# ikt-luh/Demo-Learned-Point-Cloud-Compression

Hardware: AMD Instinct MI355X
Metric: point-cloud frames/sec encode+decode @1M pts (higher is better)
Workload: dtype f32

## Files before the change

### demo-learned-point-cloud-compression_amd/csrc/codec.hip

```cpp
#include "common.h"

#include <string.h>

#include <algorithm>
#include <atomic>
#include <chrono>
#include <deque>
#include <exception>
#include <new>
#include <map>
#include <memory>
#include <string>
#include <condition_variable>
#include <functional>
#include <mutex>
#include <thread>
#include <vector>

namespace {

double now_s() {
  return std::chrono::duration<double>(std::chrono::steady_clock::now().time_since_epoch()).count();
}

// ... 652 lines not shown
};

int rans_encode_grow(const int32_t* sym, const int32_t* idx, int64_t n, const Tensor* cdf, const Tensor* len,
                     const Tensor* off, std::vector<uint8_t>* out) {
  int64_t cap = 2 * n + 4096, got = 0;
  int rc = PCC_OK;
  for (int attempt = 0; attempt < 2; ++attempt) {
    out->resize((size_t)cap);
    rc = pcc_rans_encode(sym, idx, n, cdf->i32(), (int)cdf->dims[1], len->i32(), off->i32(), (int)cdf->dims[0],
                         out->data(), cap, &got);
    if (rc != PCC_E_NOMEM) break;
    cap = 48 * n + 4096;
  }
  if (rc == PCC_OK) out->resize((size_t)got);
  return rc;
}

}


static void warm_copy_paths(pcc_codec* cd) {
  hipStream_t st = cd->ctx->stream;
  const size_t big = (size_t)1 << 20;
  uint8_t *d = nullptr, *h = nullptr;
  if (hipMalloc((void**)&d, 2 * big) != hipSuccess) return;
  if (hipHostMalloc((void**)&h, 2 * big, hipHostMallocDefault) == hipSuccess) {
    for (int rep = 0; rep < 2; ++rep) {
      for (size_t bytes : {(size_t)64, (size_t)4096, (size_t)65536, big}) {
        for (int k = 0; k < 4; ++k) {
          (void)hipMemcpyAsync(h + (size_t)k * (big / 4), d + (size_t)k * (big / 4), std::min(bytes, big / 4), hipMemcpyDeviceToHost, st);
          (void)hipMemcpyAsync(d + big + (size_t)k * (big / 4), h + big + (size_t)k * (big / 4), std::min(bytes, big / 4),
                               hipMemcpyHostToDevice, st);
        }
        (void)hipMemcpy2DAsync(h, big / 4, d, big / 4, std::min(bytes, big / 4), 3, hipMemcpyDeviceToHost, st);
        (void)hipMemcpy2DAsync(h + big, big / 4, d + big, big / 4, std::min(bytes, big / 4) / 2 + 1, 3, hipMemcpyDeviceToHost, st);
      }
      (void)hipMemsetAsync(d, 0, 4096, st);
      (void)hipMemcpyAsync(d + big, d, 65536, hipMemcpyDeviceToDevice, st);
    }
    (void)hipStreamSynchronize(st);
    (void)hipHostFree(h);
  }
  (void)hipFree(d);
  (void)hipGetLastError();
}

extern "C" pcc_codec* pcc_codec_create(const void* h_ckpt, size_t n, int device, void* stream) {
  if (!h_ckpt || n < 8 || memcmp(h_ckpt, "PCCW", 4) != 0) {
    pcc_set_error("pcc_codec_create: not a PCCW checkpoint blob");
    return nullptr;
  }
  pcc_ctx* ctx = pcc_create(device, stream);
  if (!ctx) return nullptr;
  pcc_codec* cd = new pcc_codec();
  cd->ctx = ctx;
  cd->device = device;
  cd->blob.assign((const uint8_t*)h_ckpt, (const uint8_t*)h_ckpt + n);
  const uint8_t* p = cd->blob.data();
  size_t pos = 4;
  auto fail = [&](const char* why) -> pcc_codec* {
    pcc_set_error("pcc_codec_create: malformed checkpoint (%s)", why);
    pcc_destroy(cd->ctx);
    delete cd;
    return nullptr;
  };
  uint32_t count;
  memcpy(&count, p + pos, 4);
  pos += 4;
  for (uint32_t i = 0; i < count; ++i) {
// ... 508 lines not shown
    return PCC_OK;
  }
};

struct EncodeCall {
  pcc_codec* cd;
  pcc_ctx* ctx;
  hipStream_t st;
  const double* h_q;
  int n_frames, n_q, cy, cz;
  bool v1 = false;
  pcc_ctx* side = nullptr;
  double ts[8] = {0, 0, 0, 0, 0, 0, 0, 0};
  Feat x, y, z, z_hat, gp;
  View yv, zv;
  int64_t ny = 0, nz = 0;
  float* ys_f = nullptr;
  int32_t* zsym_dev = nullptr;
  const std::vector<int64_t>* yoffs = nullptr;
  std::vector<uint64_t> root_keys;
  std::vector<int64_t> counts[3];
  GeoSlotEncoder geo;
  int64_t cap_y = 0, cap_z = 0;
  long long* d_lens = nullptr;
  hipEvent_t z_done = nullptr;
  const Tensor *eb_cdf = nullptr, *eb_len = nullptr, *eb_off = nullptr;
  const Tensor *gc_cdf = nullptr, *gc_len = nullptr, *gc_off = nullptr;
  std::vector<std::vector<uint8_t>> blobs, y_strings;
  std::vector<uint8_t> z_string, head_done;
  std::vector<int64_t> seek_idx;
  std::vector<std::vector<uint64_t>> seek_state;
  std::vector<std::vector<int64_t>> seek_word;
  int n_chunks = 1;
  std::vector<int64_t> bound;
  std::vector<hipEvent_t> evc;
  std::vector<int> rcq;
  std::vector<std::string> errq;
  double helper_z_s = 0;
  EncodeCall(pcc_codec* c, int nf, const double* q, int nq)
      : cd(c), ctx(c->ctx), st(c->ctx->stream), h_q(q), n_frames(nf), n_q(nq), cy(c->c_y), cz(c->c_z),
        blobs((size_t)nf), y_strings((size_t)nq), head_done((size_t)nq, 0) {}
  int unpack(int64_t n, const int32_t* d_coords, const float* d_feats, const FrameTab* frames_in, const HostFrames* host) {
    CODEC_ALLOC(keys, uint64_t, n);
    CODEC_ALLOC(flag, int32_t, 1);
    CODEC_ALLOC(perm, uint32_t, n);
    CODEC_ALLOC(f, float, 4 * n);
    PCC_HIP(hipMemsetAsync(flag, 0, 4, st));
    FrameTab ftab;
    const FrameTab* frames = frames_in;
    std::vector<UploadPiece> col_pieces;
    std::atomic<int> up_status{0};
    WorkersGuard up_guard{nullptr};
    if (host) {
      if (!cd->up_stream) {
        PCC_HIP(hipStreamCreateWithFlags(&cd->up_stream, hipStreamNonBlocking));
        PCC_HIP(hipEventCreateWithFlags(&cd->up_done, hipEventDisableTiming));
      }
      PCC_HIP(hipStreamSynchronize(cd->up_stream));
      ftab = *frames_in;
      const size_t pb = ftab.pts_i16 ? 6 : 12, cb = 12;
      char* dp = (char*)cd->pool.alloc((size_t)n * pb + 256 * (size_t)ftab.nf);
      char* dc = (char*)cd->pool.alloc((size_t)n * cb + 256 * (size_t)ftab.nf);
      if (!dp || !dc) return PCC_E_NOMEM;
      std::vector<UploadPiece> pt_pieces;
      size_t po = 0, co = 0;
      for (int f = 0; f < ftab.nf; ++f) {
// ... 168 lines not shown
    for (int attempt = 0; attempt < 2; ++attempt) {
      if (attempt == 1) {
        cap_y = pcc_rans_dev_bound(per);
        cap_z = pcc_rans_dev_bound(nzs);
      }
      PCC_TRY(cd->pin_ysym.ensure((size_t)cap_y * n_q + (size_t)cap_z + 256));
      ystreams = cd->pin_ysym.p;
      zstream = cd->pin_ysym.p + (size_t)cap_y * n_q;
      PCC_TRY(pcc_rans_encode_dev_async(ctx, cd->gc_dev, sym32, idx8, 1, per, n_q, ystreams, cap_y, d_lens, attempt));
      if (attempt == 0 && z_done)
        PCC_HIP(hipStreamWaitEvent(st, z_done, 0));
      else
        PCC_TRY(pcc_rans_encode_dev_async(ctx, cd->eb_dev, zsym_dev, nullptr, std::max<int64_t>(nz, 1), nzs, 1, zstream, cap_z,
                                          d_lens + n_q, attempt));
      PCC_HIP(hipMemcpyAsync(h_lens, d_lens, (size_t)(n_q + 1) * 8, hipMemcpyDeviceToHost, st));
      if (attempt == 0) PCC_TRY(geo.finish(true, blobs));
      PCC_HIP(hipStreamSynchronize(st));
      bool fits = true;
      for (int q = 0; q <= n_q; ++q) fits &= h_lens[q] >= 0;
      if (fits) break;
      PCC_REQUIRE(attempt == 0, PCC_E_NOMEM, "pcc_encode_gop: a coded stream exceeds its bound");
    }
    for (int q = 0; q < n_q; ++q) y_strings[q].assign(ystreams + (size_t)q * cap_y, ystreams + (size_t)q * cap_y + h_lens[q]);
    z_string.assign(zstream, zstream + h_lens[n_q]);
    return PCC_OK;
  }
  int gaussian_v0(float* params, float* scale_d, const Tensor* tab) {
    gc_cdf = find(cd, "gaussian_conditional.quantized_cdf");
    gc_len = find(cd, "gaussian_conditional.cdf_length");
    gc_off = find(cd, "gaussian_conditional.offset");
    PCC_REQUIRE(tab && gc_cdf && gc_len && gc_off, PCC_E_ARG, "pcc_encode_gop: gaussian_conditional tables missing");
    const int ntab = (int)tab->dims[0];
    const int64_t per = (int64_t)cy * ny, tot = per * n_q;
    CODEC_ALLOC(sym16, int16_t, std::max<int64_t>(tot, 1));
    CODEC_ALLOC(idx8, uint8_t, std::max<int64_t>(tot, 1));
    CODEC_ALLOC(flag, int32_t, 1);
    PCC_TRY(cd->pin_ysym.ensure((size_t)std::max<int64_t>(tot, 1) * 4));
    PCC_TRY(cd->pin_yidx.ensure((size_t)std::max<int64_t>(tot, 1) * 4));
    PCC_HIP(hipMemsetAsync(flag, 0, 4, st));
    if (ny > 0)
      PCC_TRY(pcc_gaussian_quant16(ctx, ys_f, params, ny, cy, scale_d, n_q, cd->dev["gaussian_conditional.scale_table"],
                                   ntab, sym16, idx8, flag));
    PCC_HIP(hipMemcpyAsync(cd->pin_flag.p, flag, 4, hipMemcpyDeviceToHost, st));
    n_chunks = per >= (1 << 16) ? 4 : 1;
    bound.resize((size_t)n_chunks);
    for (int c = 0; c < n_chunks; ++c) bound[c] = (per * (n_chunks - 1 - c) / n_chunks) & ~(int64_t)63;
    evc.assign((size_t)n_chunks, nullptr);
    for (int c = 0; c < n_chunks; ++c) {
      const int64_t lo = bound[c], hi = c == 0 ? per : bound[c - 1];
      if (ny > 0 && hi > lo) {
        PCC_HIP(hipMemcpy2DAsync(cd->pin_ysym.p + (size_t)lo * 2, (size_t)per * 2, sym16 + lo, (size_t)per * 2,
                                 (size_t)(hi - lo) * 2, (size_t)n_q, hipMemcpyDeviceToHost, st));
        PCC_HIP(hipMemcpy2DAsync(cd->pin_yidx.p + (size_t)lo, (size_t)per, idx8 + lo, (size_t)per, (size_t)(hi - lo),
                                 (size_t)n_q, hipMemcpyDeviceToHost, st));
      }
      PCC_TRY(call_event(cd, &evc[c]));
      PCC_HIP(hipEventRecord(evc[c], st));
    }
    rcq.assign((size_t)n_q, PCC_OK);
    errq.assign((size_t)n_q, std::string());
    seek_indexes(per, cd->seek_points, &seek_idx);
    seek_state.assign((size_t)n_q, std::vector<uint64_t>(seek_idx.size() + 1, 0));
    seek_word.assign((size_t)n_q, std::vector<int64_t>(seek_idx.size() + 1, 0));
    int side_rc = PCC_OK;
    {
      WorkersGuard wait_all{&cd->workers};
      cd->workers.ensure(n_q);
      for (int q = 0; q < n_q; ++q) cd->workers.run(q, [this, q]() { code_quality(q); });
      side_rc = geometry_and_z();
    }
    PCC_TRY(side_rc);
    for (int q = 0; q < n_q; ++q)
      if (rcq[q] != PCC_OK) {
        pcc_set_error("pcc_encode_gop (y stream %d): %s", q, errq[q].c_str());
        return rcq[q];
      }
    if (*(int32_t*)cd->pin_flag.p == 0) return PCC_OK;
    return gaussian_int32(params, scale_d, ntab);
  }
  void code_quality(int q) {
    struct GateUser {
      hipEvent_t* ev;
      bool failed;
    };
    (void)hipSetDevice(cd->device);
    GateUser gu{evc.data(), false};
    PccRansGate gate{n_chunks, bound.data(),
                     [](void* u, int c) {
                       GateUser* g = (GateUser*)u;
                       if (hipEventSynchronize(g->ev[c]) != hipSuccess) g->failed = true;
                     },
                     &gu};
    gate.fn(&gu, 0);
    if (gu.failed) {
      rcq[q] = PCC_E_HIP;
      errq[q] = "hipEventSynchronize failed";
      return;
    }
    if (*(volatile int32_t*)cd->pin_flag.p != 0) return;
    const int64_t per = (int64_t)cy * ny;
    int64_t capq = 2 * per + 4096, got = 0;
    std::unique_ptr<uint8_t[]> ybuf;
    for (int attempt = 0; attempt < 2; ++attempt) {
      ybuf.reset(new uint8_t[(size_t)capq]);
      PccRansSeek seek{(int)seek_idx.size(), seek_idx.data(), seek_state[q].data(), seek_word[q].data()};
      rcq[q] = pcc_rans_encode16_seek((const int16_t*)cd->pin_ysym.p + (size_t)q * per, cd->pin_yidx.p + (size_t)q * per,
                                      per, gc_cdf->i32(), (int)gc_cdf->dims[1], gc_len->i32(), gc_off->i32(),
                                      (int)gc_cdf->dims[0], ybuf.get(), capq, &got, &gate, cd->gc_tables,
                                      seek_idx.empty() ? nullptr : &seek);
      if (rcq[q] != PCC_E_NOMEM) break;
      capq = 48 * per + 4096;
    }
    if (rcq[q] == PCC_OK && gu.failed) {
      rcq[q] = PCC_E_HIP;
      errq[q] = "hipEventSynchronize failed";
    } else if (rcq[q] == PCC_OK) {
      std::vector<uint8_t>& o = cd->out[q];
      o.clear();
      o.reserve((size_t)got + 65536);
      put_head(o, n_frames, q, got, 0);
      o.insert(o.end(), ybuf.get(), ybuf.get() + got);
      head_done[q] = 1;
    } else {
      errq[q] = pcc_last_error();
    }
  }
  int geometry_and_z() {
    PCC_TRY(geo.device_half(ctx));
    PCC_TRY(geo.finish(false, blobs));
    double t = now_s();
    std::vector<int32_t> idx((size_t)nz * cz);
    for (int c = 0; c < cz; ++c) std::fill(idx.begin() + (size_t)c * nz, idx.begin() + (size_t)(c + 1) * nz, c);
    PCC_TRY(rans_encode_grow((const int32_t*)cd->pin_zsym.p, idx.data(), nz * cz, eb_cdf, eb_len, eb_off, &z_string));
    helper_z_s = now_s() - t;
    return PCC_OK;
  }
  int gaussian_int32(const float* params, const float* scale_d, int ntab) {
    const int64_t per = (int64_t)cy * ny, tot = per * n_q;
    int64_t cap = 2 * per + 4096;
    std::fill(head_done.begin(), head_done.end(), 0);
    CODEC_ALLOC(sym32, int32_t, std::max<int64_t>(tot, 1));
    CODEC_ALLOC(idx32, int32_t, std::max<int64_t>(tot, 1));
// ... 991 lines not shown
```

### demo-learned-point-cloud-compression_amd/csrc/entropy.hip

```cpp
#include "common.h"

__global__ __launch_bounds__(256) void k_factorized_quant(const float* __restrict__ z, int64_t n, int c,
                                                          const float* __restrict__ med,
                                                          int32_t* __restrict__ sym,
                                                          float* __restrict__ zhat) {
  const int64_t t = (int64_t)blockIdx.x * blockDim.x + threadIdx.x;
  if (t >= n * c) return;
  const int ch = (int)(t / n);
  const int64_t i = t - (int64_t)ch * n;
  const float m = med[ch];
  const float r = rintf(__fsub_rn(z[i * c + ch], m));
  sym[t] = (int32_t)r;
  zhat[i * c + ch] = __fadd_rn(r, m);
}

__global__ __launch_bounds__(256) void k_factorized_dequant(const int32_t* __restrict__ sym, int64_t n,
                                                            int c, const float* __restrict__ med,
                                                            float* __restrict__ zhat) {
  const int64_t t = (int64_t)blockIdx.x * blockDim.x + threadIdx.x;
  if (t >= n * c) return;
  const int ch = (int)(t / n);
  const int64_t i = t - (int64_t)ch * n;
  zhat[i * c + ch] = __fadd_rn((float)sym[t], med[ch]);
}

__device__ __forceinline__ int32_t scale_index(float sc, const float* __restrict__ table, int n_tab) {
  const float s = fmaxf(sc, table[0]);
  int32_t idx = n_tab - 1;
  for (int j = 0; j < n_tab - 1; ++j) idx -= (s <= table[j]) ? 1 : 0;
  return idx;
}

constexpr int GQ_TILE = 16;
constexpr int GQ_MAX_C = 256;
static inline size_t gq_lds_bytes(int c, int planes) { return (size_t)(64 + planes * GQ_TILE * (c + 1)) * 4; }

__device__ __forceinline__ void gq_stage(const float* __restrict__ src, int64_t row0, int rows, int width, int col0, int c,
                                         float* __restrict__ dst) {
  const int lane = threadIdx.x & 63, wave = threadIdx.x >> 6, nw = blockDim.x >> 6;
  for (int r = wave; r < rows; r += nw) {
    const float* row = src + (row0 + r) * width + col0;
    for (int j = lane; j < c; j += 64) dst[r * (c + 1) + j] = row[j];
  }
}

__device__ __forceinline__ bool gq_load_table(const float* __restrict__ table, int n_tab, float* __restrict__ tab) {
  if (threadIdx.x < n_tab) tab[threadIdx.x] = table[threadIdx.x];
  __syncthreads();
  const bool ok = !((int)threadIdx.x + 1 < n_tab) || tab[threadIdx.x] <= tab[threadIdx.x + 1];
  return __syncthreads_and(ok) != 0;
}
__device__ __forceinline__ int32_t scale_index_fast(float sc, const float* __restrict__ tab, int n_tab, bool ascending) {
  if (!ascending) return scale_index(sc, tab, n_tab);
  const float s = fmaxf(sc, tab[0]);
  int lo = 0, hi = n_tab - 1;
  while (lo < hi) {
    const int mid = (lo + hi) >> 1;
    if (tab[mid] >= s) hi = mid;
    else lo = mid + 1;
  }
  return lo;
}

template <typename SymT, typename IdxT, bool CHECK16>
__global__ __launch_bounds__(256) void k_gaussian_quant_t(
    const float* __restrict__ y, const float* __restrict__ params, int64_t n, int c,
    const float* __restrict__ scale, int nq, const float* __restrict__ table, int n_tab,
    SymT* __restrict__ sym, IdxT* __restrict__ idx, int32_t* __restrict__ flag) {
  extern __shared__ float gq_lds[];
  float* tab = gq_lds;
  float* yt = gq_lds + 64;
  float* sct = yt + GQ_TILE * (c + 1);
  float* mut = sct + GQ_TILE * (c + 1);
  const bool asc = gq_load_table(table, n_tab, tab);
  const int64_t row0 = (int64_t)blockIdx.x * GQ_TILE;
  const int rows = (int)min((int64_t)GQ_TILE, n - row0);
  gq_stage(y, row0, rows, c, 0, c, yt);
  gq_stage(params, row0, rows, 2 * c, 0, c, sct);
  gq_stage(params, row0, rows, 2 * c, c, c, mut);
  __syncthreads();
  bool over = false;
  for (int e = threadIdx.x; e < GQ_TILE * c; e += blockDim.x) {
    const int ch = e / GQ_TILE, r = e - ch * GQ_TILE;
    if (r >= rows) continue;
    const float yv = yt[r * (c + 1) + ch], sc = sct[r * (c + 1) + ch], mu = mut[r * (c + 1) + ch];
    const int64_t t = (int64_t)ch * n + row0 + r;
    for (int q = 0; q < nq; ++q) {
      const float s = scale[q * c + ch];
      const float v = rintf(__fsub_rn(__fmul_rn(yv, s), __fmul_rn(mu, s)));
      if constexpr (CHECK16) over |= !(v >= -32768.0f && v <= 32767.0f);
      sym[(int64_t)q * n * c + t] = (SymT)(int32_t)v;
      idx[(int64_t)q * n * c + t] = (IdxT)scale_index_fast(__fmul_rn(sc, s), tab, n_tab, asc);
    }
  }
  if constexpr (CHECK16)
    if (over) atomicOr(flag, 1);
}

template <typename IdxT>
__global__ __launch_bounds__(256) void k_gaussian_indexes_t(const float* __restrict__ params, int64_t n, int c,
                                                            const float* __restrict__ scale,
                                                            const float* __restrict__ table, int n_tab,
                                                            IdxT* __restrict__ idx) {
  extern __shared__ float gq_lds[];
  float* tab = gq_lds;
  float* sct = gq_lds + 64;
  const bool asc = gq_load_table(table, n_tab, tab);
  const int64_t row0 = (int64_t)blockIdx.x * GQ_TILE;
  const int rows = (int)min((int64_t)GQ_TILE, n - row0);
  gq_stage(params, row0, rows, 2 * c, 0, c, sct);
  __syncthreads();
  for (int e = threadIdx.x; e < GQ_TILE * c; e += blockDim.x) {
    const int ch = e / GQ_TILE, r = e - ch * GQ_TILE;
    if (r >= rows) continue;
    idx[(int64_t)ch * n + row0 + r] = (IdxT)scale_index_fast(__fmul_rn(sct[r * (c + 1) + ch], scale[ch]), tab, n_tab, asc);
  }
}

__global__ __launch_bounds__(256) void k_gaussian_dequant(const int32_t* __restrict__ sym,
                                                          const float* __restrict__ params, int64_t n,
                                                          int c, const float* __restrict__ scale,
                                                          float bound, float off_a, float off_b,
                                                          float* __restrict__ yhat) {
  extern __shared__ float gq_lds[];
  float* sct = gq_lds + 64;
// ... 87 lines not shown
                     c, d_med, d_zhat);
  PCC_CHECK_LAUNCH();
  return PCC_OK;
}

extern "C" int pcc_gaussian_quant(pcc_ctx* ctx, const float* d_y, const float* d_params, int64_t n,
                                  int c, const float* d_scale, int q, const float* d_table, int n_tab,
                                  int32_t* d_sym, int32_t* d_idx) {
  PCC_REQUIRE(ctx && c >= 1 && c <= GQ_MAX_C && q >= 1 && n_tab >= 2 && n_tab <= 64, PCC_E_ARG,
              "pcc_gaussian_quant: bad arg (c=%d q=%d n_tab=%d)", c, q, n_tab);
  if (n <= 0) return PCC_OK;
  PCC_REQUIRE(d_y && d_params && d_scale && d_table && d_sym && d_idx, PCC_E_ARG,
              "pcc_gaussian_quant: null buffers");
  hipLaunchKernelGGL((k_gaussian_quant_t<int32_t, int32_t, false>), dim3(nblk(n, GQ_TILE)), dim3(256), gq_lds_bytes(c, 3),
                     ctx->stream, d_y, d_params, n, c, d_scale, q, d_table, n_tab, d_sym, d_idx, (int32_t*)nullptr);
  PCC_CHECK_LAUNCH();
  return PCC_OK;
}

extern "C" int pcc_gaussian_quant16(pcc_ctx* ctx, const float* d_y, const float* d_params, int64_t n,
                                    int c, const float* d_scale, int q, const float* d_table, int n_tab,
                                    int16_t* d_sym, uint8_t* d_idx, int32_t* d_flag) {
  PCC_REQUIRE(ctx && c >= 1 && c <= GQ_MAX_C && q >= 1 && n_tab >= 2 && n_tab <= 64, PCC_E_ARG,
              "pcc_gaussian_quant16: bad arg (c=%d q=%d n_tab=%d)", c, q, n_tab);
  if (n <= 0) return PCC_OK;
  PCC_REQUIRE(d_y && d_params && d_scale && d_table && d_sym && d_idx && d_flag, PCC_E_ARG,
              "pcc_gaussian_quant16: null buffers");
  hipLaunchKernelGGL((k_gaussian_quant_t<int16_t, uint8_t, true>), dim3(nblk(n, GQ_TILE)), dim3(256), gq_lds_bytes(c, 3),
                     ctx->stream, d_y, d_params, n, c, d_scale, q, d_table, n_tab, d_sym, d_idx, d_flag);
  PCC_CHECK_LAUNCH();
  return PCC_OK;
}

extern "C" int pcc_gaussian_quant_dev(pcc_ctx* ctx, const float* d_y, const float* d_params, int64_t n, int c,
                                      const float* d_scale, int q, const float* d_table, int n_tab, int32_t* d_sym,
                                      uint8_t* d_idx) {
  PCC_REQUIRE(ctx && c >= 1 && c <= GQ_MAX_C && q >= 1 && n_tab >= 2 && n_tab <= 64, PCC_E_ARG,
              "pcc_gaussian_quant_dev: bad arg (c=%d q=%d n_tab=%d)", c, q, n_tab);
  if (n <= 0) return PCC_OK;
  PCC_REQUIRE(d_y && d_params && d_scale && d_table && d_sym && d_idx, PCC_E_ARG, "pcc_gaussian_quant_dev: null buffers");
  hipLaunchKernelGGL((k_gaussian_quant_t<int32_t, uint8_t, false>), dim3(nblk(n, GQ_TILE)), dim3(256), gq_lds_bytes(c, 3),
                     ctx->stream, d_y, d_params, n, c, d_scale, q, d_table, n_tab, d_sym, d_idx, (int32_t*)nullptr);
  PCC_CHECK_LAUNCH();
  return PCC_OK;
}

extern "C" int pcc_gaussian_indexes8(pcc_ctx* ctx, const float* d_params, int64_t n, int c,
                                     const float* d_scale, const float* d_table, int n_tab,
                                     uint8_t* d_idx) {
  PCC_REQUIRE(ctx && c >= 1 && c <= GQ_MAX_C && n_tab >= 2 && n_tab <= 64, PCC_E_ARG, "pcc_gaussian_indexes8: bad arg");
  if (n <= 0) return PCC_OK;
  PCC_REQUIRE(d_params && d_scale && d_table && d_idx, PCC_E_ARG, "pcc_gaussian_indexes8: null buffers");
  hipLaunchKernelGGL((k_gaussian_indexes_t<uint8_t>), dim3(nblk(n, GQ_TILE)), dim3(256), gq_lds_bytes(c, 1), ctx->stream,
                     d_params, n, c, d_scale, d_table, n_tab, d_idx);
  PCC_CHECK_LAUNCH();
  return PCC_OK;
}

extern "C" int pcc_gaussian_indexes(pcc_ctx* ctx, const float* d_params, int64_t n, int c,
                                    const float* d_scale, const float* d_table, int n_tab,
                                    int32_t* d_idx) {
  PCC_REQUIRE(ctx && c >= 1 && c <= GQ_MAX_C && n_tab >= 2 && n_tab <= 64, PCC_E_ARG, "pcc_gaussian_indexes: bad arg");
  if (n <= 0) return PCC_OK;
  PCC_REQUIRE(d_params && d_scale && d_table && d_idx, PCC_E_ARG, "pcc_gaussian_indexes: null buffers");
  hipLaunchKernelGGL((k_gaussian_indexes_t<int32_t>), dim3(nblk(n, GQ_TILE)), dim3(256), gq_lds_bytes(c, 1), ctx->stream,
                     d_params, n, c, d_scale, d_table, n_tab, d_idx);
// ... 16 lines not shown
```

### demo-learned-point-cloud-compression_amd/csrc/rans_gate.h

```cpp
#pragma once
#include <stdint.h>
#include <vector>

struct PccRansGate {
  int n_chunks;
  const int64_t* bound;
  void (*fn)(void* user, int chunk);
  void* user;
};
struct PccRansTables;
PccRansTables* pcc_rans_tables_build(const int32_t* h_cdfs, int cdf_pitch, const int32_t* h_sizes,
                                     const int32_t* h_offsets, int n_cdf);
void pcc_rans_tables_free(PccRansTables* t);
int pcc_rans_encode16_gated(const int16_t* h_sym, const uint8_t* h_idx, int64_t n, const int32_t* h_cdfs,
                            int cdf_pitch, const int32_t* h_sizes, const int32_t* h_offsets, int n_cdf,
                            uint8_t* h_out, int64_t cap, int64_t* h_len, const PccRansGate* gate,
                            const PccRansTables* tables);
struct PccRansSeek {
  int n;
  const int64_t* index;
  uint64_t* state;
  int64_t* word;
};
int pcc_rans_encode16_seek(const int16_t* h_sym, const uint8_t* h_idx, int64_t n, const int32_t* h_cdfs,
                           int cdf_pitch, const int32_t* h_sizes, const int32_t* h_offsets, int n_cdf,
                           uint8_t* h_out, int64_t cap, int64_t* h_len, const PccRansGate* gate,
                           const PccRansTables* tables, PccRansSeek* seek);
int pcc_rans_decode8_range(const uint8_t* h_in, int64_t len, const uint8_t* h_idx, int64_t n, const int32_t* h_cdfs,
                           int cdf_pitch, const int32_t* h_sizes, const int32_t* h_offsets, int n_cdf, int32_t* h_sym,
                           const PccRansTables* tables, int64_t i_lo, int64_t i_hi, uint64_t state_in, int64_t word_in,
                           uint64_t* state_out, int64_t* word_out);
int pcc_rans_decode8_gated(const uint8_t* h_in, int64_t len, const uint8_t* h_idx, int64_t n, const int32_t* h_cdfs,
                           int cdf_pitch, const int32_t* h_sizes, const int32_t* h_offsets, int n_cdf,
                           int32_t* h_sym, const PccRansGate* gate, const PccRansTables* tables);


int pcc_octree_unpack_vec(const uint8_t* h_in, int64_t len, std::vector<int32_t>* pts, int64_t* h_level_n);
struct PccOctPart {
  std::vector<uint64_t> cells;
  int64_t level_n[16];
};
int pcc_octree_parts(const uint8_t* h_in, int64_t len, int* K, const uint8_t** part, int64_t* part_len);
int pcc_octree_unpack_part(const uint8_t* h_in, int64_t len, PccOctPart* out);
int pcc_octree_merge_parts(const uint8_t* h_in, int64_t len, PccOctPart* parts, int K, std::vector<uint64_t>* cells,
                           int64_t* h_level_n);
void pcc_octree_cells_to_points(const uint64_t* cells, int64_t n, const int32_t origin[3], int32_t* out);
int pcc_octree_join_parts(int depth, const int32_t origin[3], int64_t n_points, const std::vector<uint8_t>* parts, int K,
                          uint8_t* h_out, int64_t cap, int64_t* h_len);

struct pcc_ctx;
struct pcc_rans_dev;
int pcc_rans_encode_dev_async(pcc_ctx* ctx, const pcc_rans_dev* tables, const int32_t* d_sym, const uint8_t* d_idx,
                              int64_t idx_run, int64_t n, int n_streams, uint8_t* d_out, int64_t cap_each,
                              long long* d_lens, int attempt);

int pcc_octree2_encode(pcc_ctx* ctx, const uint64_t* d_keys, int64_t n, int key_shift, int depth, const int32_t origin[3],
                       uint8_t* h_out, int64_t cap, int64_t* h_len);
int pcc_octree2_decode(pcc_ctx* ctx, const uint8_t* h_in, int64_t len, int32_t* d_points, int32_t* h_points, int64_t cap_points,
                       int64_t* h_n_points, int64_t* h_level_n);
```

### demo-learned-point-cloud-compression_amd/csrc/rans_host.cpp

```cpp
#include <stdint.h>
#include <string.h>
#include <stdio.h>
#include <algorithm>
#include <memory>
#include <thread>
#include <vector>
#include "../../include/pcc.h"
#include "rans_gate.h"

void pcc_set_error(const char* fmt, ...);

namespace {

constexpr uint32_t kPrecision = 16;
constexpr uint32_t kBypassBits = 4;
constexpr uint32_t kMaxBypass = (1u << kBypassBits) - 1;
constexpr uint64_t kRansL = 1ull << 31;

struct Enc {
  uint64_t x;
  uint32_t* ptr;
  uint32_t* floor;
  bool overflow;

// ... 44 lines not shown
      return PCC_E_ARG;
    }
    t->base[c + 1] = t->base[c] + sizes[c] - 1;
  }
  t->ent.resize((size_t)t->base[n_cdf]);
  for (int c = 0; c < n_cdf; ++c) {
    const int32_t* cdf = cdfs + (int64_t)c * pitch;
    for (int v = 0; v < sizes[c] - 1; ++v) {
      EncSym& e = t->ent[(size_t)t->base[c] + v];
      const int64_t f = (int64_t)cdf[v + 1] - cdf[v];
      e.freq = (f >= 1 && f <= 65536) ? (uint32_t)f : 0u;
      e.bias = (uint32_t)cdf[v];
      e.cmpl = (1u << kPrecision) - e.freq;
      if (e.freq < 2) {
        e.rcp = ~0ull;
        e.rs = 0;
        e.bias += (1u << kPrecision) - 1;
      } else {
        uint32_t shift = 0;
        while (e.freq > (1u << shift)) ++shift;
        e.rcp = (uint64_t)((((unsigned __int128)1 << (shift + 63)) + e.freq - 1) / e.freq);
        e.rs = shift - 1;
      }
      e.x_max = ((kRansL >> kPrecision) << 32) * (uint64_t)e.freq;
    }
  }
  return PCC_OK;
}

template <typename SymT, typename IdxT>
int encode_stream(const SymT* sym, const IdxT* idx, int64_t n, const int32_t* cdfs, int pitch,
                  const int32_t* sizes, const int32_t* offsets, int n_cdf, uint8_t* out, int64_t cap,
                  int64_t* len, char* err, size_t errlen, const PccRansGate* gate = nullptr,
                  const EncTables* pre = nullptr, PccRansSeek* seek = nullptr) {
  size_t buf_words = (size_t)(n / 2 + n / 8) + 1024;
  std::unique_ptr<uint32_t[]> buf(new uint32_t[buf_words]);
  EncTables local;
  if (!pre) {
    const int rc = build_enc_tables(cdfs, pitch, sizes, n_cdf, &local, err, errlen);
    if (rc != PCC_OK) return rc;
    pre = &local;
  }
  const std::vector<int32_t>& base = pre->base;
  const std::vector<EncSym>& ent = pre->ent;
  for (int attempt = 0; attempt < 3; ++attempt) {
    Enc e;
    e.x = kRansL;
    e.floor = buf.get();
    e.ptr = buf.get() + buf_words;
    e.overflow = false;
    const int n_chunks = gate ? gate->n_chunks : 1;
    int sk = seek ? seek->n - 1 : -1;
    while (sk >= 0 && seek->index[sk] >= n) --sk;
    for (int ch = 0; ch < n_chunks; ++ch) {
    const int64_t c_hi = (ch == 0 ? n : gate->bound[ch - 1]) - 1, c_lo = gate ? gate->bound[ch] : 0;
    if (gate) gate->fn(gate->user, ch);
    for (int64_t i_hi = c_hi; i_hi >= c_lo;) {
    const int64_t i_lo = (sk >= 0 && seek->index[sk] > c_lo) ? std::min<int64_t>(seek->index[sk], i_hi + 1) : c_lo;
    for (int64_t i = i_hi; i >= i_lo; --i) {
      const int32_t ci = (int32_t)idx[i];
      if ((uint32_t)ci >= (uint32_t)n_cdf) {
        snprintf(err, errlen, "rans encode: index %d out of range at %lld", ci, (long long)i);
        return PCC_E_ARG;
      }
      const int32_t max_value = sizes[ci] - 2;
      int32_t value = (int32_t)sym[i] - offsets[ci];
      if ((uint32_t)value >= (uint32_t)max_value) {
        uint32_t raw;
        if (value < 0) raw = (uint32_t)(-2 * (int64_t)value - 1);
        else raw = (uint32_t)(2 * ((int64_t)value - max_value));
        value = max_value;
        const int nb = n_nibbles(raw);
        for (int j = nb - 1; j >= 0; --j) e.put_bits((raw >> (j * kBypassBits)) & kMaxBypass);
        const int full = nb / (int)kMaxBypass;
        e.put_bits((uint32_t)(nb - full * (int)kMaxBypass));
        for (int j = 0; j < full; ++j) e.put_bits(kMaxBypass);
      }
      const EncSym& es = ent[(size_t)base[ci] + value];
      if (es.freq == 0) {
        snprintf(err, errlen, "rans encode: zero frequency (cdf %d, value %d)", ci, value);
        return PCC_E_ARG;
      }
      e.put(es);
    }
    while (sk >= 0 && seek->index[sk] >= i_lo && seek->index[sk] > 0) {
      seek->state[sk] = e.x;
      seek->word[sk] = (int64_t)((buf.get() + buf_words) - e.ptr);
      --sk;
    }
    i_hi = i_lo - 1;
    }
    }
    e.emit((uint32_t)(e.x >> 32));
    e.emit((uint32_t)(e.x >> 0));
    if (e.overflow) {
      buf_words = (size_t)n * 12 + 1024;
      buf.reset(new uint32_t[buf_words]);
      continue;
    }
// ... 253 lines not shown
      cdf_pitch < 2 || n_cdf < 1 || !gate_ok(gate, n, true)) {
    pcc_set_error("pcc_rans_encode16_gated: bad argument");
    return PCC_E_ARG;
  }
  char err[256] = {0};
  const int rc = encode_stream(h_sym, h_idx, n, h_cdfs, cdf_pitch, h_sizes, h_offsets, n_cdf, h_out, cap, h_len, err,
                               sizeof(err), gate, tables ? &tables->enc : nullptr);
  if (rc != PCC_OK) pcc_set_error("pcc_rans_encode16_gated: %s", err);
  return rc;
}

int pcc_rans_encode16_seek(const int16_t* h_sym, const uint8_t* h_idx, int64_t n, const int32_t* h_cdfs,
                           int cdf_pitch, const int32_t* h_sizes, const int32_t* h_offsets, int n_cdf,
                           uint8_t* h_out, int64_t cap, int64_t* h_len, const PccRansGate* gate,
                           const PccRansTables* tables, PccRansSeek* seek) {
  if (!h_len || n < 0 || (n > 0 && (!h_sym || !h_idx)) || !h_cdfs || !h_sizes || !h_offsets || !h_out ||
      cdf_pitch < 2 || n_cdf < 1 || !gate_ok(gate, n, true)) {
    pcc_set_error("pcc_rans_encode16_seek: bad argument");
    return PCC_E_ARG;
  }
  if (seek)
    for (int k = 0; k < seek->n; ++k)
      if (!seek->index || !seek->state || !seek->word || (k > 0 && seek->index[k] < seek->index[k - 1])) {
        pcc_set_error("pcc_rans_encode16_seek: seek indexes must ascend");
        return PCC_E_ARG;
      }
  char err[256] = {0};
  const int rc = encode_stream(h_sym, h_idx, n, h_cdfs, cdf_pitch, h_sizes, h_offsets, n_cdf, h_out, cap, h_len, err,
                               sizeof(err), gate, tables ? &tables->enc : nullptr, seek);
  if (rc != PCC_OK) pcc_set_error("pcc_rans_encode16_seek: %s", err);
  return rc;
}

int pcc_rans_decode8_range(const uint8_t* h_in, int64_t len, const uint8_t* h_idx, int64_t n, const int32_t* h_cdfs,
                           int cdf_pitch, const int32_t* h_sizes, const int32_t* h_offsets, int n_cdf, int32_t* h_sym,
                           const PccRansTables* tables, int64_t i_lo, int64_t i_hi, uint64_t state_in, int64_t word_in,
                           uint64_t* state_out, int64_t* word_out) {
  if (!tables || !state_out || !word_out || !h_in || len < 8) {
    pcc_set_error("pcc_rans_decode8_range: bad argument");
    return PCC_E_ARG;
  }
  DecPos from{state_in, word_in}, to{0, 0};
  if (i_lo == 0 && word_in == 0) {
    uint32_t w[2];
    memcpy(w, h_in, 8);
    from.x = (uint64_t)w[0] | ((uint64_t)w[1] << 32);
    from.word = 2;
  }
  const int rc = decode_stream(h_in, len, h_idx, n, h_cdfs, cdf_pitch, h_sizes, h_offsets, n_cdf, h_sym,
                               "pcc_rans_decode8_range", nullptr, &tables->dec, i_lo, i_hi, &from, &to);
  *state_out = to.x;
  *word_out = to.word;
  return rc;
}

int pcc_rans_decode8_gated(const uint8_t* h_in, int64_t len, const uint8_t* h_idx, int64_t n, const int32_t* h_cdfs,
                           int cdf_pitch, const int32_t* h_sizes, const int32_t* h_offsets, int n_cdf,
                           int32_t* h_sym, const PccRansGate* gate, const PccRansTables* tables) {
  if (!gate_ok(gate, n, false)) {
    pcc_set_error("pcc_rans_decode8_gated: bad chunk table");
    return PCC_E_ARG;
  }
  return decode_stream(h_in, len, h_idx, n, h_cdfs, cdf_pitch, h_sizes, h_offsets, n_cdf, h_sym,
                       "pcc_rans_decode8", gate, tables ? &tables->dec : nullptr);
}

// ... 82 lines not shown
```

Baseline: 118.8.

## Write gaussian symbols in chunk-contiguous pieces to replace strided 2D D2H copies

```diff
diff --git a/demo-learned-point-cloud-compression_amd/csrc/codec.hip b/demo-learned-point-cloud-compression_amd/csrc/codec.hip
--- a/demo-learned-point-cloud-compression_amd/csrc/codec.hip
+++ b/demo-learned-point-cloud-compression_amd/csrc/codec.hip
@@ -708,9 +708,8 @@
           (void)hipMemcpyAsync(d + big + (size_t)k * (big / 4), h + big + (size_t)k * (big / 4), std::min(bytes, big / 4),
                                hipMemcpyHostToDevice, st);
         }
-        (void)hipMemcpy2DAsync(h, big / 4, d, big / 4, std::min(bytes, big / 4), 3, hipMemcpyDeviceToHost, st);
-        (void)hipMemcpy2DAsync(h + big, big / 4, d + big, big / 4, std::min(bytes, big / 4) / 2 + 1, 3, hipMemcpyDeviceToHost, st);
-      }
+      }
+      (void)hipMemcpyAsync(h, d, 2 * big, hipMemcpyDeviceToHost, st);
       (void)hipMemsetAsync(d, 0, 4096, st);
       (void)hipMemcpyAsync(d + big, d, 65536, hipMemcpyDeviceToDevice, st);
     }
@@ -1285,6 +1284,7 @@
   std::vector<std::vector<uint64_t>> seek_state;
   std::vector<std::vector<int64_t>> seek_word;
   int n_chunks = 1;
+  PccSymPieces pieces{};
   std::vector<int64_t> bound;
   std::vector<hipEvent_t> evc;
   std::vector<int> rcq;
@@ -1519,28 +1519,31 @@
     PCC_REQUIRE(tab && gc_cdf && gc_len && gc_off, PCC_E_ARG, "pcc_encode_gop: gaussian_conditional tables missing");
     const int ntab = (int)tab->dims[0];
     const int64_t per = (int64_t)cy * ny, tot = per * n_q;
-    CODEC_ALLOC(sym16, int16_t, std::max<int64_t>(tot, 1));
-    CODEC_ALLOC(idx8, uint8_t, std::max<int64_t>(tot, 1));
+    n_chunks = per >= (1 << 16) ? 4 : 1;
+    bound.resize((size_t)n_chunks);
+    for (int c = 0; c < n_chunks; ++c) bound[c] = (per * (n_chunks - 1 - c) / n_chunks) & ~(int64_t)63;
+    pieces.n = n_chunks;
+    int64_t piece_bytes = 0;
+    for (int c = 0; c < n_chunks; ++c) {
+      pieces.lo[c] = bound[c];
+      pieces.len[c] = (c == 0 ? per : bound[c - 1]) - bound[c];
+      pieces.base[c] = piece_bytes;
+      piece_bytes += (pieces.len[c] * 3 * n_q + 255) & ~(int64_t)255;
+    }
+    CODEC_ALLOC(symp, uint8_t, std::max<int64_t>(piece_bytes, 1));
     CODEC_ALLOC(flag, int32_t, 1);
-    PCC_TRY(cd->pin_ysym.ensure((size_t)std::max<int64_t>(tot, 1) * 4));
+    PCC_TRY(cd->pin_ysym.ensure((size_t)std::max<int64_t>(std::max(tot * 4, piece_bytes), 1)));
     PCC_TRY(cd->pin_yidx.ensure((size_t)std::max<int64_t>(tot, 1) * 4));
     PCC_HIP(hipMemsetAsync(flag, 0, 4, st));
     if (ny > 0)
-      PCC_TRY(pcc_gaussian_quant16(ctx, ys_f, params, ny, cy, scale_d, n_q, cd->dev["gaussian_conditional.scale_table"],
-                                   ntab, sym16, idx8, flag));
+      PCC_TRY(pcc_gaussian_quant16_pieces(ctx, ys_f, params, ny, cy, scale_d, n_q,
+                                          cd->dev["gaussian_conditional.scale_table"], ntab, symp, &pieces, flag));
     PCC_HIP(hipMemcpyAsync(cd->pin_flag.p, flag, 4, hipMemcpyDeviceToHost, st));
-    n_chunks = per >= (1 << 16) ? 4 : 1;
-    bound.resize((size_t)n_chunks);
-    for (int c = 0; c < n_chunks; ++c) bound[c] = (per * (n_chunks - 1 - c) / n_chunks) & ~(int64_t)63;
     evc.assign((size_t)n_chunks, nullptr);
     for (int c = 0; c < n_chunks; ++c) {
-      const int64_t lo = bound[c], hi = c == 0 ? per : bound[c - 1];
-      if (ny > 0 && hi > lo) {
-        PCC_HIP(hipMemcpy2DAsync(cd->pin_ysym.p + (size_t)lo * 2, (size_t)per * 2, sym16 + lo, (size_t)per * 2,
-                                 (size_t)(hi - lo) * 2, (size_t)n_q, hipMemcpyDeviceToHost, st));
-        PCC_HIP(hipMemcpy2DAsync(cd->pin_yidx.p + (size_t)lo, (size_t)per, idx8 + lo, (size_t)per, (size_t)(hi - lo),
-                                 (size_t)n_q, hipMemcpyDeviceToHost, st));
-      }
+      if (pieces.len[c] > 0)
+        PCC_HIP(hipMemcpyAsync(cd->pin_ysym.p + pieces.base[c], symp + pieces.base[c], (size_t)pieces.len[c] * 3 * n_q,
+                               hipMemcpyDeviceToHost, st));
       PCC_TRY(call_event(cd, &evc[c]));
       PCC_HIP(hipEventRecord(evc[c], st));
     }
@@ -1572,6 +1575,14 @@
     };
     (void)hipSetDevice(cd->device);
     GateUser gu{evc.data(), false};
+    const int16_t* sym_at[kPccSymPiecesMax];
+    const uint8_t* idx_at[kPccSymPiecesMax];
+    for (int c = 0; c < n_chunks; ++c) {
+      const uint8_t* p = cd->pin_ysym.p + pieces.base[c];
+      sym_at[c] = (const int16_t*)p + (size_t)pieces.len[c] * q;
+      idx_at[c] = p + (size_t)pieces.len[c] * (2 * n_q + q);
+    }
+    const PccRansChunks chunks{sym_at, idx_at};
     PccRansGate gate{n_chunks, bound.data(),
                      [](void* u, int c) {
                        GateUser* g = (GateUser*)u;
@@ -1591,10 +1602,9 @@
     for (int attempt = 0; attempt < 2; ++attempt) {
       ybuf.reset(new uint8_t[(size_t)capq]);
       PccRansSeek seek{(int)seek_idx.size(), seek_idx.data(), seek_state[q].data(), seek_word[q].data()};
-      rcq[q] = pcc_rans_encode16_seek((const int16_t*)cd->pin_ysym.p + (size_t)q * per, cd->pin_yidx.p + (size_t)q * per,
-                                      per, gc_cdf->i32(), (int)gc_cdf->dims[1], gc_len->i32(), gc_off->i32(),
-                                      (int)gc_cdf->dims[0], ybuf.get(), capq, &got, &gate, cd->gc_tables,
-                                      seek_idx.empty() ? nullptr : &seek);
+      rcq[q] = pcc_rans_encode16_chunks(&chunks, per, gc_cdf->i32(), (int)gc_cdf->dims[1], gc_len->i32(), gc_off->i32(),
+                                        (int)gc_cdf->dims[0], ybuf.get(), capq, &got, &gate, cd->gc_tables,
+                                        seek_idx.empty() ? nullptr : &seek);
       if (rcq[q] != PCC_E_NOMEM) break;
       capq = 48 * per + 4096;
     }
diff --git a/demo-learned-point-cloud-compression_amd/csrc/entropy.hip b/demo-learned-point-cloud-compression_amd/csrc/entropy.hip
--- a/demo-learned-point-cloud-compression_amd/csrc/entropy.hip
+++ b/demo-learned-point-cloud-compression_amd/csrc/entropy.hip
@@ -1,4 +1,5 @@
 #include "common.h"
+#include "rans_gate.h"
 
 __global__ __launch_bounds__(256) void k_factorized_quant(const float* __restrict__ z, int64_t n, int c,
                                                           const float* __restrict__ med,
@@ -62,11 +63,11 @@
   return lo;
 }
 
-template <typename SymT, typename IdxT, bool CHECK16>
+template <typename SymT, typename IdxT, bool CHECK16, bool PIECES = false>
 __global__ __launch_bounds__(256) void k_gaussian_quant_t(
     const float* __restrict__ y, const float* __restrict__ params, int64_t n, int c,
     const float* __restrict__ scale, int nq, const float* __restrict__ table, int n_tab,
-    SymT* __restrict__ sym, IdxT* __restrict__ idx, int32_t* __restrict__ flag) {
+    SymT* __restrict__ sym, IdxT* __restrict__ idx, int32_t* __restrict__ flag, PccSymPieces pc = PccSymPieces()) {
   extern __shared__ float gq_lds[];
   float* tab = gq_lds;
   float* yt = gq_lds + 64;
@@ -85,12 +86,33 @@
     if (r >= rows) continue;
     const float yv = yt[r * (c + 1) + ch], sc = sct[r * (c + 1) + ch], mu = mut[r * (c + 1) + ch];
     const int64_t t = (int64_t)ch * n + row0 + r;
+    SymT* sym_o;
+    IdxT* idx_o;
+    int64_t pitch;
+    if constexpr (PIECES) {
+      int64_t lo = pc.lo[0], base = pc.base[0];
+      pitch = pc.len[0];
+#pragma unroll
+      for (int k = 1; k < kPccSymPiecesMax; ++k)
+        if (k < pc.n && t < pc.lo[k - 1]) {
+          lo = pc.lo[k];
+          base = pc.base[k];
+          pitch = pc.len[k];
+        }
+      uint8_t* piece = (uint8_t*)sym + base;
+      sym_o = (SymT*)piece + (t - lo);
+      idx_o = (IdxT*)(piece + pitch * nq * (int64_t)sizeof(SymT)) + (t - lo);
+    } else {
+      sym_o = sym + t;
+      idx_o = idx + t;
+      pitch = n * c;
+    }
     for (int q = 0; q < nq; ++q) {
       const float s = scale[q * c + ch];
       const float v = rintf(__fsub_rn(__fmul_rn(yv, s), __fmul_rn(mu, s)));
       if constexpr (CHECK16) over |= !(v >= -32768.0f && v <= 32767.0f);
-      sym[(int64_t)q * n * c + t] = (SymT)(int32_t)v;
-      idx[(int64_t)q * n * c + t] = (IdxT)scale_index_fast(__fmul_rn(sc, s), tab, n_tab, asc);
+      sym_o[q * pitch] = (SymT)(int32_t)v;
+      idx_o[q * pitch] = (IdxT)scale_index_fast(__fmul_rn(sc, s), tab, n_tab, asc);
     }
   }
   if constexpr (CHECK16)
@@ -244,6 +266,30 @@
   return PCC_OK;
 }
 
+int pcc_gaussian_quant16_pieces(pcc_ctx* ctx, const float* d_y, const float* d_params, int64_t n, int c,
+                                const float* d_scale, int q, const float* d_table, int n_tab, uint8_t* d_out,
+                                const PccSymPieces* pieces, int32_t* d_flag) {
+  PCC_REQUIRE(ctx && c >= 1 && c <= GQ_MAX_C && q >= 1 && n_tab >= 2 && n_tab <= 64, PCC_E_ARG,
+              "pcc_gaussian_quant16_pieces: bad arg (c=%d q=%d n_tab=%d)", c, q, n_tab);
+  if (n <= 0) return PCC_OK;
+  PCC_REQUIRE(d_y && d_params && d_scale && d_table && d_out && pieces && d_flag, PCC_E_ARG,
+              "pcc_gaussian_quant16_pieces: null buffers");
+  PCC_REQUIRE(pieces->n >= 1 && pieces->n <= kPccSymPiecesMax, PCC_E_ARG, "pcc_gaussian_quant16_pieces: %d pieces", pieces->n);
+  int64_t hi = n * c, end = 0;
+  for (int p = 0; p < pieces->n; ++p) {
+    PCC_REQUIRE(pieces->len[p] >= 0 && pieces->lo[p] + pieces->len[p] == hi && pieces->base[p] >= end && pieces->base[p] % 2 == 0,
+                PCC_E_ARG, "pcc_gaussian_quant16_pieces: piece %d does not continue the tiling", p);
+    hi = pieces->lo[p];
+    end = pieces->base[p] + pieces->len[p] * 3 * q;
+  }
+  PCC_REQUIRE(hi == 0, PCC_E_ARG, "pcc_gaussian_quant16_pieces: the pieces do not reach element 0");
+  hipLaunchKernelGGL((k_gaussian_quant_t<int16_t, uint8_t, true, true>), dim3(nblk(n, GQ_TILE)), dim3(256), gq_lds_bytes(c, 3),
+                     ctx->stream, d_y, d_params, n, c, d_scale, q, d_table, n_tab, (int16_t*)d_out, (uint8_t*)nullptr, d_flag,
+                     *pieces);
+  PCC_CHECK_LAUNCH();
+  return PCC_OK;
+}
+
 extern "C" int pcc_gaussian_quant_dev(pcc_ctx* ctx, const float* d_y, const float* d_params, int64_t n, int c,
                                       const float* d_scale, int q, const float* d_table, int n_tab, int32_t* d_sym,
                                       uint8_t* d_idx) {
diff --git a/demo-learned-point-cloud-compression_amd/csrc/rans_gate.h b/demo-learned-point-cloud-compression_amd/csrc/rans_gate.h
--- a/demo-learned-point-cloud-compression_amd/csrc/rans_gate.h
+++ b/demo-learned-point-cloud-compression_amd/csrc/rans_gate.h
@@ -8,6 +8,19 @@
   void (*fn)(void* user, int chunk);
   void* user;
 };
+struct PccRansChunks {
+  const int16_t* const* sym_at;
+  const uint8_t* const* idx_at;
+};
+constexpr int kPccSymPiecesMax = 4;
+struct PccSymPieces {
+  int n;
+  int64_t lo[kPccSymPiecesMax], len[kPccSymPiecesMax], base[kPccSymPiecesMax];
+};
+struct pcc_ctx;
+int pcc_gaussian_quant16_pieces(pcc_ctx* ctx, const float* d_y, const float* d_params, int64_t n, int c,
+                                const float* d_scale, int q, const float* d_table, int n_tab, uint8_t* d_out,
+                                const PccSymPieces* pieces, int32_t* d_flag);
 struct PccRansTables;
 PccRansTables* pcc_rans_tables_build(const int32_t* h_cdfs, int cdf_pitch, const int32_t* h_sizes,
                                      const int32_t* h_offsets, int n_cdf);
@@ -26,6 +39,9 @@
                            int cdf_pitch, const int32_t* h_sizes, const int32_t* h_offsets, int n_cdf,
                            uint8_t* h_out, int64_t cap, int64_t* h_len, const PccRansGate* gate,
                            const PccRansTables* tables, PccRansSeek* seek);
+int pcc_rans_encode16_chunks(const PccRansChunks* chunks, int64_t n, const int32_t* h_cdfs, int cdf_pitch,
+                             const int32_t* h_sizes, const int32_t* h_offsets, int n_cdf, uint8_t* h_out, int64_t cap,
+                             int64_t* h_len, const PccRansGate* gate, const PccRansTables* tables, PccRansSeek* seek);
 int pcc_rans_decode8_range(const uint8_t* h_in, int64_t len, const uint8_t* h_idx, int64_t n, const int32_t* h_cdfs,
                            int cdf_pitch, const int32_t* h_sizes, const int32_t* h_offsets, int n_cdf, int32_t* h_sym,
                            const PccRansTables* tables, int64_t i_lo, int64_t i_hi, uint64_t state_in, int64_t word_in,
diff --git a/demo-learned-point-cloud-compression_amd/csrc/rans_host.cpp b/demo-learned-point-cloud-compression_amd/csrc/rans_host.cpp
--- a/demo-learned-point-cloud-compression_amd/csrc/rans_host.cpp
+++ b/demo-learned-point-cloud-compression_amd/csrc/rans_host.cpp
@@ -100,7 +100,7 @@
 int encode_stream(const SymT* sym, const IdxT* idx, int64_t n, const int32_t* cdfs, int pitch,
                   const int32_t* sizes, const int32_t* offsets, int n_cdf, uint8_t* out, int64_t cap,
                   int64_t* len, char* err, size_t errlen, const PccRansGate* gate = nullptr,
-                  const EncTables* pre = nullptr, PccRansSeek* seek = nullptr) {
+                  const EncTables* pre = nullptr, PccRansSeek* seek = nullptr, const PccRansChunks* at = nullptr) {
   size_t buf_words = (size_t)(n / 2 + n / 8) + 1024;
   std::unique_ptr<uint32_t[]> buf(new uint32_t[buf_words]);
   EncTables local;
@@ -123,16 +123,19 @@
     for (int ch = 0; ch < n_chunks; ++ch) {
     const int64_t c_hi = (ch == 0 ? n : gate->bound[ch - 1]) - 1, c_lo = gate ? gate->bound[ch] : 0;
     if (gate) gate->fn(gate->user, ch);
+    const SymT* csym = at ? (const SymT*)at->sym_at[ch] : sym;
+    const IdxT* cidx = at ? (const IdxT*)at->idx_at[ch] : idx;
+    const int64_t c_at = at ? c_lo : 0;
     for (int64_t i_hi = c_hi; i_hi >= c_lo;) {
     const int64_t i_lo = (sk >= 0 && seek->index[sk] > c_lo) ? std::min<int64_t>(seek->index[sk], i_hi + 1) : c_lo;
     for (int64_t i = i_hi; i >= i_lo; --i) {
-      const int32_t ci = (int32_t)idx[i];
+      const int32_t ci = (int32_t)cidx[i - c_at];
       if ((uint32_t)ci >= (uint32_t)n_cdf) {
         snprintf(err, errlen, "rans encode: index %d out of range at %lld", ci, (long long)i);
         return PCC_E_ARG;
       }
       const int32_t max_value = sizes[ci] - 2;
-      int32_t value = (int32_t)sym[i] - offsets[ci];
+      int32_t value = (int32_t)csym[i - c_at] - offsets[ci];
       if ((uint32_t)value >= (uint32_t)max_value) {
         uint32_t raw;
         if (value < 0) raw = (uint32_t)(-2 * (int64_t)value - 1);
@@ -452,6 +455,30 @@
   return rc;
 }
 
+int pcc_rans_encode16_chunks(const PccRansChunks* chunks, int64_t n, const int32_t* h_cdfs, int cdf_pitch,
+                             const int32_t* h_sizes, const int32_t* h_offsets, int n_cdf, uint8_t* h_out, int64_t cap,
+                             int64_t* h_len, const PccRansGate* gate, const PccRansTables* tables, PccRansSeek* seek) {
+  bool ok = h_len && n >= 0 && chunks && chunks->sym_at && chunks->idx_at && h_cdfs && h_sizes && h_offsets && h_out &&
+            cdf_pitch >= 2 && n_cdf >= 1 && gate && gate_ok(gate, n, true);
+  for (int c = 0; ok && c < gate->n_chunks; ++c)
+    ok = (c == 0 ? n : gate->bound[c - 1]) == gate->bound[c] || (chunks->sym_at[c] && chunks->idx_at[c]);
+  if (!ok) {
+    pcc_set_error("pcc_rans_encode16_chunks: bad argument");
+    return PCC_E_ARG;
+  }
+  if (seek)
+    for (int k = 0; k < seek->n; ++k)
+      if (!seek->index || !seek->state || !seek->word || (k > 0 && seek->index[k] < seek->index[k - 1])) {
+        pcc_set_error("pcc_rans_encode16_chunks: seek indexes must ascend");
+        return PCC_E_ARG;
+      }
+  char err[256] = {0};
+  const int rc = encode_stream((const int16_t*)nullptr, (const uint8_t*)nullptr, n, h_cdfs, cdf_pitch, h_sizes, h_offsets,
+                               n_cdf, h_out, cap, h_len, err, sizeof(err), gate, tables ? &tables->enc : nullptr, seek, chunks);
+  if (rc != PCC_OK) pcc_set_error("pcc_rans_encode16_chunks: %s", err);
+  return rc;
+}
+
 int pcc_rans_decode8_range(const uint8_t* h_in, int64_t len, const uint8_t* h_idx, int64_t n, const int32_t* h_cdfs,
                            int cdf_pitch, const int32_t* h_sizes, const int32_t* h_offsets, int n_cdf, int32_t* h_sym,
                            const PccRansTables* tables, int64_t i_lo, int64_t i_hi, uint64_t state_in, int64_t word_in,
```

After: 117.9. About the same (-0.7%).
